# stefan01/Fusion-Method-for-Video-Frame-Interpolation

Measured on NVIDIA B200. Metric: interpolated_1080p_frames_per_s, higher is better.
Workload: dtype f32

## Files before the change

### fusion-method-for-video-frame-interpolation_b200/csrc/common.cuh

```cuda
#pragma once
#include <cuda_runtime.h>
#include <stdint.h>
#include <stdio.h>
#include <string>

#include "fvfi.h"

namespace fvfi {

void set_error(const char* fmt, ...);
void note_launch();

#define FVFI_CHECK_ARG(cond, ...)            \
    do {                                     \
        if (!(cond)) {                       \
            ::fvfi::set_error(__VA_ARGS__);  \
            return FVFI_EINVAL;              \
        }                                    \
    } while (0)

#define FVFI_CUDA(expr)                                                                   \
    do {                                                                                  \
        cudaError_t _e = (expr);                                                          \
        if (_e != cudaSuccess) {                                                          \
// ... 27 lines not shown
__host__ __device__ __forceinline__ int ceil_div(int a, int b) { return (a + b - 1) / b; }

__device__ __forceinline__ float ld_stream(const float* p) {
    float v;
    asm("ld.global.nc.L1::no_allocate.f32 %0, [%1];" : "=f"(v) : "l"(p));
    return v;
}
__device__ __forceinline__ void st_stream(float* p, float v) {
    asm volatile("st.global.L1::no_allocate.f32 [%0], %1;" ::"l"(p), "f"(v) : "memory");
}
__device__ __forceinline__ float4 ld_stream4(const float4* p) {
    float4 v;
    asm("ld.global.nc.L1::no_allocate.v4.f32 {%0,%1,%2,%3}, [%4];"
                 : "=f"(v.x), "=f"(v.y), "=f"(v.z), "=f"(v.w)
                 : "l"(p));
    return v;
}
__device__ __forceinline__ void st_stream4(float4* p, float4 v) {
    asm volatile("st.global.L1::no_allocate.v4.f32 [%0], {%1,%2,%3,%4};" ::"l"(p), "f"(v.x), "f"(v.y),
                 "f"(v.z), "f"(v.w)
                 : "memory");
}

__host__ __device__ __forceinline__ void bilinear_src(int o, float scale, int align_corners, int n_in, int& i0, int& i1, float& l) {
    const float f = align_corners ? scale * (float)o : fmaxf(scale * ((float)o + 0.5f) - 0.5f, 0.f);
    i0 = min((int)f, n_in - 1);
    i1 = min(i0 + 1, n_in - 1);
    l = f - (float)i0;
}
__host__ __device__ __forceinline__ float bilinear_scale(int n_in, int n_out, int align_corners) {
    if (align_corners) return n_out > 1 ? (float)(n_in - 1) / (float)(n_out - 1) : 0.f;
    return (float)n_in / (float)n_out;
}
__device__ __forceinline__ float bilerp(float hy, float hx, float ly, float lx, float a, float b, float c, float d) {
    return fmaf(ly, fmaf(lx, d, hx * c), hy * fmaf(lx, b, hx * a));
}
}
```

### fusion-method-for-video-frame-interpolation_b200/csrc/conv_tc.cu

```cuda
#include <cuda_fp16.h>

#include <algorithm>
#include <atomic>
#include <cstdlib>
#include <mutex>
#include <type_traits>

#include "common.cuh"

namespace fvfi {

constexpr int CV_KCHUNKS = 4;
constexpr int CV_UMAX = 12;
constexpr int CV_HDR = 32;
constexpr int CV_X_SHIFT = 4;
constexpr int CV_ROWS = 16;
constexpr int CV_LOADER_WARPS = 8;
constexpr int CV_LOADERS = 32 * CV_LOADER_WARPS;
constexpr int CV_EPI_WARPS = 4;
constexpr int CV_EPI_THREADS = 32 * CV_EPI_WARPS;
constexpr int CV_PRODUCER_WARP = CV_LOADER_WARPS + CV_EPI_WARPS;
constexpr int CV_MMA_WARP = CV_PRODUCER_WARP + 1;
constexpr int CV_THREADS = CV_LOADERS + CV_EPI_THREADS + 128;
constexpr int CV_REGS_LOADER = 152, CV_REGS_EPI = 144, CV_REGS_MISC = 56;
// ... 3 lines not shown
constexpr int CV_MAX_BSTAGES = 4;
constexpr unsigned CV_SPIN_LIMIT = 200u * 1000u * 1000u;

enum { ACT_NONE = 0, ACT_RELU = 1, ACT_ELU = 2, ACT_TANH = 3, ACT_SIGMOID = 4, ACT_SOFTMAX = 5 };
enum { PAD_ZERO = 0, PAD_REFLECT = 1 };
enum { PREC_TF32X3 = 0, PREC_F16X3 = 1 };
__host__ __device__ constexpr int cv_cpk(int prec) { return prec == PREC_F16X3 ? 8 : 4; }
__host__ __device__ constexpr int cv_chunk(int prec) { return CV_KCHUNKS * cv_cpk(prec); }

struct ConvArgs {
    const float* x;
    const float* wpack;
    const float* hdr;
    int* overflow;
    const float* bias;
    float* y;
    int B, H, W, Cin, Cout, Npad, KH, KW, pad_mode, act;
    int ldx, ldy;
    int out_nchw;
    int cout_store;
    int MT, RW, RH, NPIX;
    int KCS;
    int nchunks, last_ksteps, astages, bstages, tmem_cols;
    int wide, tcols;
    int nacc;
    int tiles_x, tiles_y, ntiles;
    unsigned a_stage_bytes, b_stage_bytes;
    const float* res;
    int ldr;
    int up, Hs, Ws, up_align;
    float up_sy, up_sx;
    const float* x2;
    int ldx2, up_chunks;
};

__device__ __forceinline__ unsigned smem_u32(const void* p) { return (unsigned)__cvta_generic_to_shared(p); }

__device__ __forceinline__ void mbar_init(unsigned long long* bar, unsigned count) {
    asm volatile("mbarrier.init.shared::cta.b64 [%0], %1;" ::"r"(smem_u32(bar)), "r"(count));
}
__device__ __forceinline__ void mbar_arrive(unsigned long long* bar) {
    asm volatile("mbarrier.arrive.shared::cta.b64 _, [%0];" ::"r"(smem_u32(bar)) : "memory");
}
__device__ __forceinline__ void mbar_expect_tx(unsigned long long* bar, unsigned bytes) {
    asm volatile("mbarrier.arrive.expect_tx.shared::cta.b64 _, [%0], %1;" ::"r"(smem_u32(bar)), "r"(bytes) : "memory");
}
__device__ __forceinline__ void mbar_wait(unsigned long long* bar, unsigned parity) {
    const unsigned addr = smem_u32(bar);
    unsigned done = 0, spins = 0;
    while (true) {
        asm volatile(
            "{\n\t.reg .pred p;\n\t"
            "mbarrier.try_wait.parity.shared::cta.b64 p, [%1], %2;\n\t"
            "selp.u32 %0, 1, 0, p;\n\t}"
            : "=r"(done)
            : "r"(addr), "r"(parity)
            : "memory");
        if (done) break;
        if (++spins > CV_SPIN_LIMIT) __trap();
    }
}
__device__ __forceinline__ void bulk_g2s(void* dst, const void* src, unsigned bytes, unsigned long long* bar) {
    asm volatile("cp.async.bulk.shared::cluster.global.mbarrier::complete_tx::bytes [%0], [%1], %2, [%3];" ::"r"(smem_u32(dst)),
                 "l"(src), "r"(bytes), "r"(smem_u32(bar))
                 : "memory");
}
// ... 69 lines not shown
__device__ __forceinline__ void tc_ld_wait() { asm volatile("tcgen05.wait::ld.sync.aligned;" ::: "memory"); }
__device__ __forceinline__ void tc_ld16(unsigned taddr, float* v) {
    unsigned r[16];
    asm volatile(
        "tcgen05.ld.sync.aligned.32x32b.x16.b32 {%0,%1,%2,%3,%4,%5,%6,%7,%8,%9,%10,%11,%12,%13,%14,%15}, [%16];"
        : "=r"(r[0]), "=r"(r[1]), "=r"(r[2]), "=r"(r[3]), "=r"(r[4]), "=r"(r[5]), "=r"(r[6]), "=r"(r[7]), "=r"(r[8]),
          "=r"(r[9]), "=r"(r[10]), "=r"(r[11]), "=r"(r[12]), "=r"(r[13]), "=r"(r[14]), "=r"(r[15])
        : "r"(taddr));
    asm volatile("tcgen05.wait::ld.sync.aligned;" ::: "memory");
#pragma unroll
    for (int i = 0; i < 16; ++i) v[i] = __uint_as_float(r[i]);
}

__device__ __forceinline__ unsigned long long make_desc(unsigned saddr, unsigned lbo_bytes, unsigned sbo_bytes) {
    unsigned long long d = 0;
    d |= (unsigned long long)((saddr >> 4) & 0x3fffu);
    d |= (unsigned long long)((lbo_bytes >> 4) & 0x3fffu) << 16;
    d |= (unsigned long long)((sbo_bytes >> 4) & 0x3fffu) << 32;
    d |= 1ull << 46;
    return d;
}

__device__ __forceinline__ void ldg256(const float* p, float* v) {
    asm volatile("ld.global.nc.v8.f32 {%0,%1,%2,%3,%4,%5,%6,%7}, [%8];"
                 : "=f"(v[0]), "=f"(v[1]), "=f"(v[2]), "=f"(v[3]), "=f"(v[4]), "=f"(v[5]), "=f"(v[6]), "=f"(v[7])
                 : "l"(p));
}
__device__ __forceinline__ void stg256(float* p, const float* v) {
    asm volatile("st.global.v8.f32 [%0], {%1,%2,%3,%4,%5,%6,%7,%8};" ::"l"(p), "f"(v[0]), "f"(v[1]), "f"(v[2]), "f"(v[3]),
                 "f"(v[4]), "f"(v[5]), "f"(v[6]), "f"(v[7])
                 : "memory");
}

__device__ __forceinline__ float to_tf32_rna(float x) {
    unsigned r;
    asm("cvt.rna.tf32.f32 %0, %1;" : "=r"(r) : "f"(x));
    return __uint_as_float(r);
}

__device__ __forceinline__ float fast_tanh(float v) {
    const float t = __expf(2.f * fminf(fmaxf(v, -15.f), 15.f));
    return __fdividef(t - 1.f, t + 1.f);
}
__device__ __forceinline__ float fast_sigmoid(float v) { return __fdividef(1.f, 1.f + __expf(-fmaxf(v, -80.f))); }
template <int ACT>
__device__ __forceinline__ float apply_act(float v) {
    switch (ACT) {
        case ACT_RELU: return fmaxf(v, 0.f);
        case ACT_ELU: return v > 0.f ? v : __expf(v) - 1.f;
        case ACT_TANH: return fast_tanh(v);
        case ACT_SIGMOID: return fast_sigmoid(v);
        default: return v;
    }
}

__device__ __forceinline__ int reflect101(int i, int n) {
    if (n == 1) return 0;
    const int period = 2 * (n - 1);
    int m = i % period;
    if (m < 0) m += period;
    return m < n ? m : period - m;
}

__global__ void conv_weight_scale_kernel(const float* __restrict__ w, size_t count, float* __restrict__ hdr, int prec) {
    __shared__ float red[32];
    float m = 0.f;
// ... 41 lines not shown
        size_t t = q;
        const int e = (int)(t % CPK); t /= CPK;
        const int n = (int)(t % Npad); t /= Npad;
        const int lo = (int)(t % 2); t /= 2;
        const int kc = (int)(t % CV_KCHUNKS); t /= CV_KCHUNKS;
        const int tap = (int)(t % taps); t /= taps;
        const int chunk = (int)t;
        const int c = chunk * (CV_KCHUNKS * CPK) + kc * CPK + e;
        float v = 0.f;
        if (n < Cout && c < Cin) v = w[(((size_t)n * Cin + c) * KH + tap / KW) * KW + tap % KW];
        if (PREC == PREC_F16X3) {
            v *= wscale;
            const __half hi = __float2half_rn(v);
            out16[q] = lo ? __float2half_rn(v - __half2float(hi)) : hi;
        } else {
            unsigned hb;
            asm("cvt.rna.tf32.f32 %0, %1;" : "=r"(hb) : "f"(v));
            const float hi = __uint_as_float(hb);
            out32[q] = lo ? (v - hi) : hi;
        }
    }
}

struct TileCoord { int img, y0, x0; };
__device__ __forceinline__ TileCoord tile_coord(const ConvArgs& A, int tile) {
    TileCoord t;
    const int bx = tile % A.tiles_x, r = tile / A.tiles_x;
    t.x0 = bx * 8 * A.MT;
    t.y0 = (r % A.tiles_y) * CV_ROWS;
    t.img = r / A.tiles_y;
    return t;
}

template <int ACT, int PREC>
__global__ void __launch_bounds__(CV_THREADS, 1) conv_split_kernel(const ConvArgs A) {
    extern __shared__ __align__(128) unsigned char smem_raw[];
    unsigned char* a_base = smem_raw;
    unsigned char* b_base = a_base + (size_t)A.astages * A.a_stage_bytes;
    unsigned long long* bars = (unsigned long long*)(b_base + (size_t)A.bstages * A.b_stage_bytes);
    unsigned long long* a_full = bars;
    unsigned long long* a_empty = bars + CV_MAX_ASTAGES;
    unsigned long long* b_full = bars + 2 * CV_MAX_ASTAGES;
    unsigned long long* b_empty = b_full + CV_MAX_BSTAGES;
    unsigned long long* acc_full = b_empty + CV_MAX_BSTAGES;
    unsigned long long* acc_empty = acc_full + 2;
    unsigned* tmem_ptr = (unsigned*)(acc_empty + 2);
    int* pixoff = (int*)(tmem_ptr + 2);
    float* bias_s = (float*)(((size_t)(pixoff + A.NPIX) + 15) & ~(size_t)15);
    float2* up_w = (float2*)(bias_s + 256);
    int* up_d = (int*)(up_w + A.NPIX);
    int* up_off = up_d + A.NPIX;

    const int warp = threadIdx.x >> 5, lane = threadIdx.x & 31;
    const int taps = A.KH * A.KW;
    const unsigned a_half = A.a_stage_bytes / 2;
    const int nacc = A.nacc;
    const unsigned acc_cols = (unsigned)(A.MT * A.tcols);

    if (threadIdx.x == 0) {
        for (int s = 0; s < A.astages; ++s) { mbar_init(&a_full[s], CV_LOADERS); mbar_init(&a_empty[s], 1); }
        for (int s = 0; s < A.bstages; ++s) { mbar_init(&b_full[s], 1); mbar_init(&b_empty[s], 1); }
        for (int s = 0; s < 2; ++s) { mbar_init(&acc_full[s], 1); mbar_init(&acc_empty[s], CV_EPI_THREADS); }
        asm volatile("fence.mbarrier_init.release.cluster;" ::: "memory");
    }
    for (int n = threadIdx.x; n < A.Npad; n += CV_THREADS) bias_s[n] = (A.bias && n < A.Cout) ? __ldg(A.bias + n) : 0.f;
    if (warp == CV_MMA_WARP) {
        asm volatile("tcgen05.alloc.cta_group::1.sync.aligned.shared::cta.b32 [%0], %1;" ::"r"(smem_u32(tmem_ptr)), "r"(A.tmem_cols));
        asm volatile("tcgen05.relinquish_alloc_permit.cta_group::1.sync.aligned;");
    }
    tc_fence_before();
    __syncthreads();
    tc_fence_after();
    const unsigned tmem = *tmem_ptr;

    if (warp >= CV_LOADER_WARPS && warp < CV_PRODUCER_WARP) {
        if (CV_REGS_EPI > CV_REGS_LAUNCH) asm volatile("setmaxnreg.inc.sync.aligned.u32 %0;" ::"n"(CV_REGS_EPI));
        else asm volatile("setmaxnreg.dec.sync.aligned.u32 %0;" ::"n"(CV_REGS_EPI));
        const float oscale = __ldg(A.hdr);
        const bool vec_out = (A.cout_store & 3) == 0 && (A.ldy & 3) == 0 && ((((size_t)A.y) & 15) == 0);
        const bool vec_out8 = (A.cout_store & 7) == 0 && (A.ldy & 7) == 0 && ((((size_t)A.y) & 31) == 0);
        const size_t plane = (size_t)A.H * A.W;
        const int quarter = warp & 3;
        const int m = quarter * 32 + lane;
        const bool res_vec = A.res && (A.Cout & 15) == 0 && (A.ldr & 7) == 0 && ((((size_t)A.res) & 31) == 0);
// ... 162 lines not shown
                    emit_at(a0, a1);
                    if (k + 1 < nblk) {
                        tc_ld_wait();
                        if (k + 2 < nblk) issue_at(a0, a1);
                        emit_at(b0, b1);
                    }
                }
            }
            tc_fence_before();
            mbar_arrive(&acc_empty[buf]);
        };

        {
            int j = 0;
            for (int tile = blockIdx.x; tile < A.ntiles; tile += gridDim.x, ++j) epilogue(j, tile_coord(A, tile));
        }
    } else if (warp < CV_LOADER_WARPS) {
        asm volatile("setmaxnreg.inc.sync.aligned.u32 %0;" ::"n"(CV_REGS_LOADER));
        const int padT = A.KH / 2, padL = A.KW / 2;
        constexpr int CPK = cv_cpk(PREC);
        constexpr int CHUNK = cv_chunk(PREC);
        const int cshift = A.up ? A.up_chunks * CHUNK : 0;
        const float* xd = (A.up && A.x2) ? A.x2 : A.x;
        const int ldd = (A.up && A.x2) ? A.ldx2 : A.ldx, cind = A.Cin - cshift;
        const int cin4 = (cind + 3) & ~3;
        const bool vec = ((ldd & 3) == 0) && (ldd >= cin4) && ((((size_t)xd) & 15) == 0);
        const int cin8 = (cind + 7) & ~7;
        const bool vec8 = ((ldd & 7) == 0) && (ldd >= cin8) && ((((size_t)xd) & 31) == 0);
        const int cin4u = A.up ? ((min(A.Cin, cshift) + 3) & ~3) : 0;
        const float xs = (float)(1 << CV_X_SHIFT);
        float amax = 0.f;
        int g = 0;

        constexpr int UMAX = CV_UMAX;
        float v[UMAX][CPK];
        auto chunk_shape = [&](int c, int& ksh) {
            ksh = (c == A.nchunks - 1 && A.last_ksteps == 1) ? 1 : 2;
            return A.NPIX << ksh;
        };
        auto issue = [&](int c, const float* X) {
            int ksh;
            const int total = chunk_shape(c, ksh);
            const int kmask = (1 << ksh) - 1, cbase = c * CHUNK - cshift;
#pragma unroll
            for (int u = 0; u < UMAX; ++u) {
                const int q = threadIdx.x + u * CV_LOADERS;
#pragma unroll
                for (int e = 0; e < CPK; ++e) v[u][e] = 0.f;
                if (q < total) {
                    const int pix = q >> ksh, ch = cbase + (q & kmask) * CPK;
                    const int off = pixoff[pix];
                    if (off >= 0 && ch < cin4) {
                        const float* p = X + (size_t)off * ldd + ch;
                        if (vec8 && CPK == 8 && ch + 8 <= cin8) {
                            ldg256(p, v[u]);
                        } else if (vec) {
#pragma unroll
                            for (int e = 0; e < CPK; e += 4) {
                                if (ch + e < cin4) {
                                    const float4 t = __ldg((const float4*)(p + e));
                                    v[u][e] = t.x; v[u][e + 1] = t.y; v[u][e + 2] = t.z; v[u][e + 3] = t.w;
                                }
                            }
                        } else {
#pragma unroll
                            for (int e = 0; e < CPK; ++e)
                                if (ch + e < cind) v[u][e] = __ldg(p + e);
                        }
                    }
                }
            }
        };
        auto finish = [&](int c) {
            const int s = g % A.astages;
            if (g >= A.astages) mbar_wait(&a_empty[s], ((g / A.astages) - 1) & 1);
            ++g;
            float4* hi = (float4*)(a_base + (size_t)s * A.a_stage_bytes);
            float4* lo = (float4*)(a_base + (size_t)s * A.a_stage_bytes + a_half);
            int ksh;
            const int total = chunk_shape(c, ksh);
            const int kmask = (1 << ksh) - 1;
#pragma unroll
            for (int u = 0; u < UMAX; ++u) {
                const int q = threadIdx.x + u * CV_LOADERS;
                if (q < total) {
                    const int o = (q & kmask) * A.KCS + (q >> ksh);
                    if (PREC == PREC_F16X3) {
                        unsigned hw[4], lw[4];
#pragma unroll
                        for (int e = 0; e < 8; e += 2) {
                            const float x0 = v[u][e] * xs, x1 = v[u][e + 1] * xs;
                            amax = fmaxf(amax, fmaxf(fabsf(x0), fabsf(x1)));
                            const __half2 h = __floats2half2_rn(x0, x1);
                            const float2 hf = __half22float2(h);
                            const __half2 l = __floats2half2_rn(x0 - hf.x, x1 - hf.y);
                            hw[e >> 1] = *(const unsigned*)&h;
                            lw[e >> 1] = *(const unsigned*)&l;
                        }
                        hi[o] = make_float4(__uint_as_float(hw[0]), __uint_as_float(hw[1]), __uint_as_float(hw[2]), __uint_as_float(hw[3]));
                        lo[o] = make_float4(__uint_as_float(lw[0]), __uint_as_float(lw[1]), __uint_as_float(lw[2]), __uint_as_float(lw[3]));
                    } else {
                        float4 h;
                        h.x = to_tf32_rna(v[u][0]); h.y = to_tf32_rna(v[u][1]); h.z = to_tf32_rna(v[u][2]); h.w = to_tf32_rna(v[u][3]);
                        hi[o] = h;
                        lo[o] = make_float4(v[u][0] - h.x, v[u][1] - h.y, v[u][2] - h.z, v[u][3] - h.w);
                    }
                }
            }
            fence_async_smem();
            mbar_arrive(&a_full[s]);
        };
        auto load_cpk = [&](const float* p, float* dst) {
            if (CPK == 8) {
                ldg256(p, dst);
            } else {
                const float4 t = __ldg((const float4*)p);
                dst[0] = t.x; dst[1] = t.y; dst[2] = t.z; dst[3] = t.w;
            }
        };
        auto stage_up = [&](int c, const float* X) {
            const int s = g % A.astages;
            if (g >= A.astages) mbar_wait(&a_empty[s], ((g / A.astages) - 1) & 1);
            ++g;
            float4* hi = (float4*)(a_base + (size_t)s * A.a_stage_bytes);
            float4* lo = (float4*)(a_base + (size_t)s * A.a_stage_bytes + a_half);
            int ksh;
            const int total = chunk_shape(c, ksh) >> 1;
            const int kmask = (1 << ksh) - 1, cbase = c * CHUNK;
            auto put = [&](int o, const float* w) {
                if (PREC == PREC_F16X3) {
                    unsigned hw[4], lw[4];
#pragma unroll
                    for (int e = 0; e < 8; e += 2) {
                        const float x0 = w[e] * xs, x1 = w[e + 1] * xs;
                        amax = fmaxf(amax, fmaxf(fabsf(x0), fabsf(x1)));
                        const __half2 h = __floats2half2_rn(x0, x1);
                        const float2 hf = __half22float2(h);
                        const __half2 l = __floats2half2_rn(x0 - hf.x, x1 - hf.y);
                        hw[e >> 1] = *(const unsigned*)&h;
                        lw[e >> 1] = *(const unsigned*)&l;
                    }
                    hi[o] = make_float4(__uint_as_float(hw[0]), __uint_as_float(hw[1]), __uint_as_float(hw[2]), __uint_as_float(hw[3]));
                    lo[o] = make_float4(__uint_as_float(lw[0]), __uint_as_float(lw[1]), __uint_as_float(lw[2]), __uint_as_float(lw[3]));
                } else {
                    float4 h;
                    h.x = to_tf32_rna(w[0]); h.y = to_tf32_rna(w[1]); h.z = to_tf32_rna(w[2]); h.w = to_tf32_rna(w[3]);
                    hi[o] = h;
                    lo[o] = make_float4(w[0] - h.x, w[1] - h.y, w[2] - h.z, w[3] - h.w);
                }
            };
            for (int q = threadIdx.x; q < total; q += CV_LOADERS) {
                const int pix = (q >> ksh) << 1, kg = q & kmask, ch = cbase + kg * CPK;
                float a0[CPK], b0[CPK], c0[CPK], d0[CPK], a1[CPK], b1[CPK], c1[CPK], d1[CPK];
#pragma unroll
                for (int e = 0; e < CPK; ++e) a0[e] = b0[e] = c0[e] = d0[e] = a1[e] = b1[e] = c1[e] = d1[e] = 0.f;
                const bool chok = ch < cin4u;
                const int off0 = chok ? up_off[pix] : -1, off1 = chok ? up_off[pix + 1] : -1;
                const int e0 = up_d[pix], e1 = up_d[pix + 1];
                const float2 w0 = up_w[pix], w1 = up_w[pix + 1];
                const int kind = (off0 >= 0 && off1 == off0 && e1 == e0) ? 0
                               : (off0 >= 0 && off1 == off0 + (e0 & 1) && (e1 >> 1) == (e0 >> 1)) ? 1 : 2;
                if (off0 >= 0) {
                    const float* p = X + (size_t)off0 * A.ldx + ch;
                    const size_t dx = (size_t)(e0 & 1) * A.ldx, dy = (size_t)(e0 >> 1) * A.ldx;
                    load_cpk(p, a0); load_cpk(p + dx, b0); load_cpk(p + dy, c0); load_cpk(p + dy + dx, d0);
                }
                if (off1 >= 0 && kind != 0) {
                    const float* p = X + (size_t)off1 * A.ldx + ch;
                    const size_t dx = (size_t)(e1 & 1) * A.ldx, dy = (size_t)(e1 >> 1) * A.ldx;
                    if (kind == 2) { load_cpk(p, a1); load_cpk(p + dy, c1); }
                    load_cpk(p + dx, b1); load_cpk(p + dy + dx, d1);
                }
                float w[CPK];
                {
                    const float ly = w0.x, lx = w0.y, hy = 1.f - ly, hx = 1.f - lx;
#pragma unroll
                    for (int e = 0; e < CPK; ++e) w[e] = bilerp(hy, hx, ly, lx, a0[e], b0[e], c0[e], d0[e]);
                    put(kg * A.KCS + pix, w);
                }
                {
                    const float ly = w1.x, lx = w1.y, hy = 1.f - ly, hx = 1.f - lx;
#pragma unroll
                    for (int e = 0; e < CPK; ++e) {
                        const float a = kind == 0 ? a0[e] : kind == 1 ? b0[e] : a1[e], cc = kind == 0 ? c0[e] : kind == 1 ? d0[e] : c1[e];
                        const float b = kind == 0 ? b0[e] : b1[e], d = kind == 0 ? d0[e] : d1[e];
                        w[e] = off1 >= 0 ? bilerp(hy, hx, ly, lx, a, b, cc, d) : 0.f;
                    }
                    put(kg * A.KCS + pix + 1, w);
                }
            }
            fence_async_smem();
            mbar_arrive(&a_full[s]);
        };
        auto map_tile = [&](const TileCoord& T) {
            asm volatile("bar.sync 1, %0;" ::"n"(CV_LOADERS) : "memory");
            for (int pix = threadIdx.x; pix < A.NPIX; pix += CV_LOADERS) {
                const int r = pix / A.RW, cc = pix - r * A.RW;
                int gy = T.y0 + r - padT, gx = T.x0 + cc - padL;
                bool ok = true;
                if (A.pad_mode == PAD_REFLECT) {
                    gy = reflect101(gy, A.H);
                    gx = reflect101(gx, A.W);
                } else {
                    ok = (gy >= 0 && gy < A.H && gx >= 0 && gx < A.W);
                }
                if (A.up) {
                    int y0 = 0, y1 = 0, x0 = 0, x1 = 0;
                    float ly = 0.f, lx = 0.f;
                    if (ok) {
                        bilinear_src(gy, A.up_sy, A.up_align, A.Hs, y0, y1, ly);
                        bilinear_src(gx, A.up_sx, A.up_align, A.Ws, x0, x1, lx);
                    }
                    up_off[pix] = ok ? y0 * A.Ws + x0 : -1;
                    up_w[pix] = make_float2(ly, lx);
                    up_d[pix] = ((y1 - y0) * A.Ws) * 2 + (x1 - x0);
                }
                pixoff[pix] = ok ? gy * A.W + gx : -1;
            }
            asm volatile("bar.sync 1, %0;" ::"n"(CV_LOADERS) : "memory");
        };

        TileCoord curT = tile_coord(A, blockIdx.x), nextT = curT;
        const float* X = xd + (size_t)curT.img * A.H * A.W * ldd;
        if (A.up) {
            for (int tile = blockIdx.x; tile < A.ntiles; tile += gridDim.x) {
                const TileCoord T = tile_coord(A, tile);
                const float* Xu = A.x + (size_t)T.img * A.Hs * A.Ws * A.ldx;
                X = xd + (size_t)T.img * A.H * A.W * ldd;
                map_tile(T);
                for (int c = 0; c < A.up_chunks; ++c) stage_up(c, Xu);
                for (int c = A.up_chunks; c < A.nchunks; ++c) {
                    issue(c, X);
                    finish(c);
                }
            }
        } else {
        if ((int)blockIdx.x < A.ntiles) {
            map_tile(curT);
            issue(0, X);
        }
        for (int tile = blockIdx.x; tile < A.ntiles; tile += gridDim.x) {
            for (int c = 0; c < A.nchunks; ++c) {
                finish(c);
                if (c + 1 < A.nchunks) {
                    issue(c + 1, X);
                } else if (tile + (int)gridDim.x < A.ntiles) {
                    nextT = tile_coord(A, tile + gridDim.x);
                    X = xd + (size_t)nextT.img * A.H * A.W * ldd;
                    map_tile(nextT);
                    issue(0, X);
                }
            }
            curT = nextT;
        }
        }
        if (PREC == PREC_F16X3 && !(amax <= 65504.f) && A.overflow) atomicOr(A.overflow, 1);
    } else {
      asm volatile("setmaxnreg.dec.sync.aligned.u32 %0;" ::"n"(CV_REGS_MISC));
      if (warp == CV_PRODUCER_WARP) {
        if (lane == 0) {
            int it = 0;
            for (int tile = blockIdx.x; tile < A.ntiles; tile += gridDim.x)
                for (int c = 0; c < A.nchunks; ++c)
                    for (int tp = 0; tp < taps; ++tp, ++it) {
                        const int s = it % A.bstages;
                        if (it >= A.bstages) mbar_wait(&b_empty[s], ((it / A.bstages) - 1) & 1);
// ... 74 lines not shown
        asm volatile("tcgen05.dealloc.cta_group::1.sync.aligned.b32 %0, %1;" ::"r"(tmem), "r"(A.tmem_cols));
    }
}

static int conv_geometry(ConvArgs& a, int prec, size_t* smem_bytes) {
    const int chunk = cv_chunk(prec);
    a.Npad = (a.Cout + 15) & ~15;
    FVFI_CHECK_ARG(a.Npad >= 16 && a.Npad <= 256, "conv: Cout %d not supported (1..256 per launch)", a.Cout);
    a.nchunks = (a.Cin + chunk - 1) / chunk;
    a.last_ksteps = (a.Cin - (a.nchunks - 1) * chunk) > chunk / 2 ? 2 : 1;
    a.b_stage_bytes = (unsigned)a.Npad * CV_KCHUNKS * 16u * 2u;
    const int taps = a.KH * a.KW;
    const size_t budget = 222 * 1024;
    static const int force_mt = [] { const char* e = getenv("FVFI_CONV_MT"); return e ? atoi(e) : 0; }();
    for (int mt = 4; mt >= 1; mt >>= 1) {
        if (force_mt && mt > force_mt) continue;
        a.wide = (a.Npad <= 32 && a.act != ACT_SOFTMAX) ? 1 : 0;
        a.tcols = a.wide ? 2 * a.Npad : a.Npad;
        if (mt * a.tcols > 512) continue;
        if (mt > 1 && 2 * mt * a.tcols > 512) continue;
        if (mt > 1 && 8 * (mt / 2) >= a.W) continue;
        a.MT = mt;
        a.nacc = (2 * mt * a.tcols <= 512) ? 2 : 1;
        a.RW = 8 * mt + a.KW - 1;
        a.RH = CV_ROWS + a.KH - 1;
        a.NPIX = a.RW * a.RH;
#ifdef FVFI_CONV_NO_KCS_PAD
        a.KCS = a.NPIX;
#else
        a.KCS = a.NPIX + ((2 - a.NPIX) & 7);
#endif
        a.a_stage_bytes = (unsigned)a.KCS * CV_KCHUNKS * 16u * 2u;
        if (a.NPIX * CV_KCHUNKS > CV_LOADERS * CV_UMAX) continue;
        const size_t misc = 512 + (size_t)a.NPIX * 4 + 1024 + 16 + (a.up ? (size_t)a.NPIX * 16 : 0);
        const int min_b = std::min(2, a.nchunks * taps);
        if (misc + 2 * (size_t)a.a_stage_bytes + (size_t)min_b * a.b_stage_bytes > budget) continue;
        int bs = std::min(CV_MAX_BSTAGES, std::max(min_b, (int)((budget - misc - 2 * (size_t)a.a_stage_bytes) / a.b_stage_bytes)));
        int as = (int)((budget - misc - (size_t)bs * a.b_stage_bytes) / a.a_stage_bytes);
        a.bstages = bs;
        a.astages = std::max(2, std::min(CV_MAX_ASTAGES, as));
        int cols = 32;
        while (cols < a.nacc * mt * a.tcols) cols <<= 1;
        a.tmem_cols = cols;
        *smem_bytes = misc + (size_t)a.astages * a.a_stage_bytes + (size_t)a.bstages * a.b_stage_bytes;
        a.tiles_x = ceil_div(a.W, 8 * mt);
        a.tiles_y = ceil_div(a.H, CV_ROWS);
        a.ntiles = a.tiles_x * a.tiles_y * a.B;
        return FVFI_OK;
    }
    set_error("conv: no tile configuration fits (Cout %d, kernel %dx%d)", a.Cout, a.KH, a.KW);
    return FVFI_EINVAL;
}

static int* overflow_flag() {
    static std::mutex mu;
    static std::atomic<int*> flags[FVFI_MAX_DEVICES];
    const int dev = current_device();
    if (dev < 0 || dev >= FVFI_MAX_DEVICES) return nullptr;
    int* p = flags[dev].load(std::memory_order_acquire);
    if (p) return p;
    std::lock_guard<std::mutex> lock(mu);
    p = flags[dev].load(std::memory_order_relaxed);
    if (!p) {
        if (cudaMalloc(&p, sizeof(int)) != cudaSuccess) return nullptr;
        cudaMemset(p, 0, sizeof(int));
        flags[dev].store(p, std::memory_order_release);
    }
    return p;
}

template <int PREC>
static void (*pick_kernel(int activation))(const ConvArgs) {
    switch (activation) {
        case ACT_RELU: return conv_split_kernel<ACT_RELU, PREC>;
        case ACT_ELU: return conv_split_kernel<ACT_ELU, PREC>;
        case ACT_TANH: return conv_split_kernel<ACT_TANH, PREC>;
        case ACT_SIGMOID: return conv_split_kernel<ACT_SIGMOID, PREC>;
        case ACT_SOFTMAX: return conv_split_kernel<ACT_SOFTMAX, PREC>;
        default: return conv_split_kernel<ACT_NONE, PREC>;
    }
}

}

using namespace fvfi;

extern "C" size_t fvfi_conv2d_packed_weight_floats(int Cout, int Cin, int KH, int KW, int precision) {
    const int Npad = (Cout + 15) & ~15;
    const int chunk = cv_chunk(precision);
    const int nchunks = (Cin + chunk - 1) / chunk;
    return (size_t)CV_HDR + (size_t)nchunks * KH * KW * 2 * CV_KCHUNKS * Npad * 4;
}

extern "C" int fvfi_conv2d_pack_weights(const float* weight_oihw, float* packed, int Cout, int Cin, int KH, int KW,
                                        int precision, void* stream) {
    FVFI_CHECK_ARG(weight_oihw && packed && Cout > 0 && Cin > 0 && KH > 0 && KW > 0, "conv_pack_weights: bad argument");
    FVFI_CHECK_ARG(precision == PREC_TF32X3 || precision == PREC_F16X3, "conv_pack_weights: precision must be 0 (3xTF32) or 1 (3xFP16)");
    const int Npad = (Cout + 15) & ~15;
    const int chunk = cv_chunk(precision);
    const int nchunks = (Cin + chunk - 1) / chunk;
    const size_t total = (size_t)nchunks * KH * KW * 2 * CV_KCHUNKS * Npad * cv_cpk(precision);
    const unsigned blocks = (unsigned)((total + 255) / 256 > 4096 ? 4096 : (total + 255) / 256);
    cudaStream_t s = (cudaStream_t)stream;
    conv_weight_scale_kernel<<<1, 1024, 0, s>>>(weight_oihw, (size_t)Cout * Cin * KH * KW, packed, precision);
    FVFI_LAUNCH_CHECK();
    if (precision == PREC_F16X3)
        conv_pack_weights_kernel<PREC_F16X3><<<blocks, 256, 0, s>>>(weight_oihw, packed, Cout, Cin, KH, KW, Npad, nchunks);
    else
        conv_pack_weights_kernel<PREC_TF32X3><<<blocks, 256, 0, s>>>(weight_oihw, packed, Cout, Cin, KH, KW, Npad, nchunks);
    FVFI_LAUNCH_CHECK();
    return FVFI_OK;
}
// ... 18 lines not shown
                                         const float* residual, int residual_pixel_stride, float* y, int y_pixel_stride, int B, int H,
                                         int W, int Cin, int Cout, int KH, int KW, int pad_mode, int activation, int out_nchw,
                                         int precision, void* stream) {
    return fvfi_conv2d_nhwc_upsampled(x, x_pixel_stride, 0, 0, 0, nullptr, 0, 0, packed_weight, bias, residual, residual_pixel_stride, y,
                                      y_pixel_stride, B, H, W, Cin, Cout, KH, KW, pad_mode, activation, out_nchw, precision, stream);
}

extern "C" int fvfi_conv2d_nhwc_upsampled(const float* x, int x_pixel_stride, int Hs, int Ws, int align_corners, const float* x_direct,
                                          int x_direct_pixel_stride, int cin_upsampled,
                                          const float* packed_weight, const float* bias, const float* residual,
                                          int residual_pixel_stride, float* y, int y_pixel_stride, int B, int H, int W, int Cin,
                                          int Cout, int KH, int KW, int pad_mode, int activation, int out_nchw, int precision,
                                          void* stream) {
    FVFI_CHECK_ARG(!residual || (activation != ACT_SOFTMAX && residual_pixel_stride >= Cout),
                   "conv2d: a residual needs a pixel stride >= Cout and no softmax");
    FVFI_CHECK_ARG(x && packed_weight && y, "conv2d: null pointer");
    FVFI_CHECK_ARG(B > 0 && H > 0 && W > 0 && Cin > 0 && Cout > 0 && B <= 65535, "conv2d: bad dimension");
    FVFI_CHECK_ARG((KH == 1 || KH == 3 || KH == 5) && KW == KH, "conv2d: kernel must be 1x1, 3x3 or 5x5");
    FVFI_CHECK_ARG(pad_mode == PAD_ZERO || pad_mode == PAD_REFLECT, "conv2d: pad_mode must be 0 (zero) or 1 (reflect)");
    FVFI_CHECK_ARG(pad_mode != PAD_REFLECT || (H > KH / 2 && W > KW / 2), "conv2d: reflect padding needs H,W > pad");
    FVFI_CHECK_ARG(activation >= 0 && activation <= 5, "conv2d: bad activation");
    FVFI_CHECK_ARG(activation != ACT_SOFTMAX || Cout <= 256, "conv2d: softmax needs all channels in one call");
    FVFI_CHECK_ARG(precision == PREC_TF32X3 || precision == PREC_F16X3, "conv2d: precision must be 0 (3xTF32) or 1 (3xFP16)");
    ConvArgs a{};
    a.x = x; a.hdr = packed_weight; a.wpack = packed_weight + CV_HDR; a.bias = bias; a.y = y;
    a.ldx = x_pixel_stride; a.ldy = y_pixel_stride; a.out_nchw = (out_nchw == 1) ? 1 : 0;
    a.res = residual; a.ldr = residual_pixel_stride;
    a.up = (Hs > 0 || Ws > 0) ? 1 : 0;
    if (a.up) {
        const int cpk = cv_cpk(precision), cin_r = (Cin + cpk - 1) / cpk * cpk;
        FVFI_CHECK_ARG(Hs > 0 && Ws > 0 && (size_t)Hs * Ws < (1u << 30), "conv2d: bad source size %dx%d for the upsampling loader", Hs, Ws);
        FVFI_CHECK_ARG((x_pixel_stride % cpk) == 0 && (x_direct || x_pixel_stride >= cin_r) && ((size_t)x % (4 * cpk)) == 0,
                       "conv2d: the upsampling loader needs an aligned source whose pixel stride is a multiple of %d and >= %d", cpk, cin_r);
        a.Hs = Hs; a.Ws = Ws; a.up_align = align_corners ? 1 : 0;
        a.up_sy = bilinear_scale(Hs, H, a.up_align);
        a.up_sx = bilinear_scale(Ws, W, a.up_align);
        const int chunk = cv_chunk(precision);
        a.up_chunks = (Cin + chunk - 1) / chunk;
        if (x_direct) {
            FVFI_CHECK_ARG(cin_upsampled > 0 && cin_upsampled < Cin && (cin_upsampled % chunk) == 0,
                           "conv2d: the upsampled part of a two-source input must be a multiple of %d channels (got %d of %d)", chunk,
                           cin_upsampled, Cin);
            FVFI_CHECK_ARG(x_direct_pixel_stride >= Cin - cin_upsampled, "conv2d: x_direct pixel stride smaller than its channel count");
            a.x2 = x_direct; a.ldx2 = x_direct_pixel_stride; a.up_chunks = cin_upsampled / chunk;
        }
    } else {
        FVFI_CHECK_ARG(!x_direct, "conv2d: x_direct needs an upsampled first source");
    }
    a.cout_store = (out_nchw == 2) ? ((Cout + 15) & ~15) : Cout;
    FVFI_CHECK_ARG(out_nchw >= 0 && out_nchw <= 2, "conv2d: output layout must be 0 (NHWC), 1 (NCHW) or 2 (NHWC, zero-padded channels)");
    FVFI_CHECK_ARG(out_nchw != 2 || y_pixel_stride >= a.cout_store, "conv2d: padded NHWC output needs a pixel stride >= round16(Cout)");
    a.overflow = (precision == PREC_F16X3) ? overflow_flag() : nullptr;
    FVFI_CHECK_ARG(x_pixel_stride >= (x_direct ? cin_upsampled : Cin) && (out_nchw || y_pixel_stride >= Cout),
                   "conv2d: pixel stride smaller than channel count");
    a.B = B; a.H = H; a.W = W; a.Cin = Cin; a.Cout = Cout; a.KH = KH; a.KW = KW; a.pad_mode = pad_mode; a.act = activation;
    size_t smem = 0;
    if (int rc = conv_geometry(a, precision, &smem)) return rc;
    const int nsm = sm_count();
    dim3 grid((unsigned)std::min(a.ntiles, nsm > 0 ? nsm : 148), 1, 1);
    void (*kern)(const ConvArgs) = (precision == PREC_F16X3) ? pick_kernel<PREC_F16X3>(activation) : pick_kernel<PREC_TF32X3>(activation);
    FVFI_SMEM_OPT_IN(kern, smem);
    kern<<<grid, CV_THREADS, smem, (cudaStream_t)stream>>>(a);
    FVFI_LAUNCH_CHECK();
    return FVFI_OK;
}
```

### fusion-method-for-video-frame-interpolation_b200/fvfi/conv.py

```python
import os

import torch

from . import _lib

PRECISIONS = {"tf32x3": 0, "f16x3": 1}
precision = PRECISIONS[os.environ.get("FVFI_CONV_PREC", "f16x3")]
range_check = True
_guard_depth = 0


def overflow_pending():
    import torch as _t
    _t.cuda.current_stream().synchronize()
    return _lib.lib().fvfi_conv2d_overflow_count() > 0


def check_overflow():
    if precision == PRECISIONS["f16x3"] and overflow_pending():
        raise FloatingPointError("fvfi.conv: activation beyond the 3xFP16 range (|x| > 4094); use conv.forced_precision('tf32x3')")


class forced_precision:

# ... 140 lines not shown
            return x
    return x.contiguous(memory_format=torch.channels_last)


fuse_upsample = True


def conv2d(x, weight, bias=None, padding_mode="zeros", act=None, out=None, nchw_out=False, pad_out=False, residual=None,
           upsample=None, x_direct=None):
    if not x.is_cuda:
        raise NotImplementedError("fvfi.conv.conv2d: CUDA tensors only")
    if torch.is_grad_enabled() and (x.requires_grad or weight.requires_grad or (bias is not None and bias.requires_grad)):
        assert upsample is None, "conv2d(upsample=...) is an inference form"
        assert out is None and not nchw_out and not pad_out and residual is None and act != "softmax", \
            "conv2d under autograd supports the plain NHWC form (bias + relu / elu / tanh / sigmoid)"
        return _ConvTC.apply(x, weight, bias, padding_mode, act)
    B, Cin, H, W = x.shape
    Cout, Cin_w, KH, KW = weight.shape
    xd, cin_up = None, 0
    if x_direct is not None:
        chunk = 32 if precision == PRECISIONS["f16x3"] else 16
        assert upsample is not None and Cin % chunk == 0 and Cin + x_direct.shape[1] >= Cin_w > Cin
        assert tuple(x_direct.shape[2:]) == tuple(int(v) for v in upsample[0]) and x_direct.shape[0] == B
        xd, cin_up = to_nhwc(x_direct.float()), Cin
        Cin = Cin_w
    assert Cin >= Cin_w and KH == KW and KH in (1, 3, 5)
    Cin = Cin_w
    xc = to_nhwc(x.float())
    assert xc.stride(1) == 1
    ldx = xc.stride(3)
    Hs = Ws = align = 0
    if upsample is not None:
        cpk = 8 if precision == PRECISIONS["f16x3"] else 4
        if ldx % cpk or ldx < ((cin_up or Cin) + cpk - 1) // cpk * cpk or xc.data_ptr() % (4 * cpk):
            up = resize_bilinear(xc, tuple(upsample[0]), bool(upsample[1]))
            if xd is not None:
                up = torch.cat((up[:, :cin_up], xd), 1)
            return conv2d(up, weight, bias, padding_mode, act, out, nchw_out, pad_out, residual)
        Hs, Ws, align = H, W, int(bool(upsample[1]))
        H, W = (int(v) for v in upsample[0])
    if (upsample is None and KH == 1 and Cout <= 8 and Cin % 8 == 0 and Cin <= 128 and ldx % 8 == 0 and xc.data_ptr() % 32 == 0
            and act != "softmax" and out is None and not nchw_out and not pad_out and residual is None):
        return _conv1x1_direct(xc, weight, bias, act)
    if out is None:
        out = torch.empty((B, (Cout + 15) // 16 * 16 if pad_out else Cout, H, W), dtype=torch.float32, device=x.device,
                          memory_format=torch.contiguous_format if nchw_out else torch.channels_last)
    ldy = Cout if nchw_out else out.stride(3)
    if nchw_out:
        assert out.is_contiguous() and Cout <= 256 and not pad_out
    if pad_out:
        assert Cout <= 256
    L = _lib.lib()
    pad_mode = {"zeros": 0, "reflect": 1}[padding_mode]
    b = None if bias is None else bias.detach().contiguous().float()
    rc = None
    if residual is not None:
        assert not nchw_out and act != "softmax" and tuple(residual.shape) == (B, Cout, H, W)
        rc = to_nhwc(residual.float())
    with torch.cuda.device(x.device):
        parts = _packed(weight)
        if timing is not None:
            e0, e1 = torch.cuda.Event(enable_timing=True), torch.cuda.Event(enable_timing=True)
            e0.record()
        for (o, n, buf) in parts:
            _lib.check(L.fvfi_conv2d_nhwc_upsampled(xc.data_ptr(), ldx, Hs, Ws, align, None if xd is None else xd.data_ptr(),
                                                    0 if xd is None else xd.stride(3), cin_up, buf.data_ptr(),
                                                    None if b is None else b.data_ptr() + 4 * o,
# ... 198 lines not shown
```

Before: 24.51.

## Restructure fused-upsample conv loader to walk column pairs down row strips reusing source rows

The bilinear-upsample loader in the tensor-core conv kernel is rewritten. The per-pixel offset and weight tables in shared memory are removed. Each loader thread now handles a pair of output columns over a strip of rows, caching horizontally interpolated source rows so they are reused across consecutive output rows, and prefetching the next rows into L1. The kernel is templated on UP, which shrinks the register array in the upsample variant, and the direct-channel chunks are issued in sub-batches. A new guard requires the source to be no larger than the output, otherwise it falls back to a separate resize.

New measurement: 24.85 (median of 6 runs). 1.4% higher.

```diff
diff --git a/fusion-method-for-video-frame-interpolation_b200/csrc/common.cuh b/fusion-method-for-video-frame-interpolation_b200/csrc/common.cuh
--- a/fusion-method-for-video-frame-interpolation_b200/csrc/common.cuh
+++ b/fusion-method-for-video-frame-interpolation_b200/csrc/common.cuh
@@ -83,7 +83,9 @@
     if (align_corners) return n_out > 1 ? (float)(n_in - 1) / (float)(n_out - 1) : 0.f;
     return (float)n_in / (float)n_out;
 }
+__device__ __forceinline__ float bilerp_row(float hx, float lx, float a, float b) { return fmaf(lx, b, hx * a); }
+__device__ __forceinline__ float bilerp_rows(float hy, float ly, float r0, float r1) { return fmaf(ly, r1, hy * r0); }
 __device__ __forceinline__ float bilerp(float hy, float hx, float ly, float lx, float a, float b, float c, float d) {
-    return fmaf(ly, fmaf(lx, d, hx * c), hy * fmaf(lx, b, hx * a));
+    return bilerp_rows(hy, ly, bilerp_row(hx, lx, a, b), bilerp_row(hx, lx, c, d));
 }
 }
diff --git a/fusion-method-for-video-frame-interpolation_b200/csrc/conv_tc.cu b/fusion-method-for-video-frame-interpolation_b200/csrc/conv_tc.cu
--- a/fusion-method-for-video-frame-interpolation_b200/csrc/conv_tc.cu
+++ b/fusion-method-for-video-frame-interpolation_b200/csrc/conv_tc.cu
@@ -59,6 +59,7 @@
     float up_sy, up_sx;
     const float* x2;
     int ldx2, up_chunks;
+    int up_seg, up_nseg;
 };
 
 __device__ __forceinline__ unsigned smem_u32(const void* p) { return (unsigned)__cvta_generic_to_shared(p); }
@@ -194,6 +195,8 @@
                  : "memory");
 }
 
+__device__ __forceinline__ void prefetch_l1(const float* p) { asm volatile("prefetch.global.L1 [%0];" ::"l"(p)); }
+
 __device__ __forceinline__ float to_tf32_rna(float x) {
     unsigned r;
     asm("cvt.rna.tf32.f32 %0, %1;" : "=r"(r) : "f"(x));
@@ -301,7 +304,7 @@
     return t;
 }
 
-template <int ACT, int PREC>
+template <int ACT, int PREC, bool UP>
 __global__ void __launch_bounds__(CV_THREADS, 1) conv_split_kernel(const ConvArgs A) {
     extern __shared__ __align__(128) unsigned char smem_raw[];
     unsigned char* a_base = smem_raw;
@@ -316,9 +319,6 @@
     unsigned* tmem_ptr = (unsigned*)(acc_empty + 2);
     int* pixoff = (int*)(tmem_ptr + 2);
     float* bias_s = (float*)(((size_t)(pixoff + A.NPIX) + 15) & ~(size_t)15);
-    float2* up_w = (float2*)(bias_s + 256);
-    int* up_d = (int*)(up_w + A.NPIX);
-    int* up_off = up_d + A.NPIX;
 
     const int warp = threadIdx.x >> 5, lane = threadIdx.x & 31;
     const int taps = A.KH * A.KW;
@@ -547,19 +547,19 @@
         float amax = 0.f;
         int g = 0;
 
-        constexpr int UMAX = CV_UMAX;
+        constexpr int UMAX = UP ? CV_UMAX / 2 : CV_UMAX;
         float v[UMAX][CPK];
         auto chunk_shape = [&](int c, int& ksh) {
             ksh = (c == A.nchunks - 1 && A.last_ksteps == 1) ? 1 : 2;
             return A.NPIX << ksh;
         };
-        auto issue = [&](int c, const float* X) {
+        auto issue = [&](int c, const float* X, int q0 = 0) {
             int ksh;
             const int total = chunk_shape(c, ksh);
             const int kmask = (1 << ksh) - 1, cbase = c * CHUNK - cshift;
 #pragma unroll
             for (int u = 0; u < UMAX; ++u) {
-                const int q = threadIdx.x + u * CV_LOADERS;
+                const int q = q0 + threadIdx.x + u * CV_LOADERS;
 #pragma unroll
                 for (int e = 0; e < CPK; ++e) v[u][e] = 0.f;
                 if (q < total) {
@@ -586,10 +586,34 @@
                 }
             }
         };
-        auto finish = [&](int c) {
-            const int s = g % A.astages;
-            if (g >= A.astages) mbar_wait(&a_empty[s], ((g / A.astages) - 1) & 1);
-            ++g;
+        auto put = [&](float4* hi, float4* lo, int o, const float* w) {
+            if (PREC == PREC_F16X3) {
+                unsigned hw[4], lw[4];
+#pragma unroll
+                for (int e = 0; e < 8; e += 2) {
+                    const float x0 = w[e] * xs, x1 = w[e + 1] * xs;
+                    amax = fmaxf(amax, fmaxf(fabsf(x0), fabsf(x1)));
+                    const __half2 h = __floats2half2_rn(x0, x1);
+                    const float2 hf = __half22float2(h);
+                    const __half2 l = __floats2half2_rn(x0 - hf.x, x1 - hf.y);
+                    hw[e >> 1] = *(const unsigned*)&h;
+                    lw[e >> 1] = *(const unsigned*)&l;
+                }
+                hi[o] = make_float4(__uint_as_float(hw[0]), __uint_as_float(hw[1]), __uint_as_float(hw[2]), __uint_as_float(hw[3]));
+                lo[o] = make_float4(__uint_as_float(lw[0]), __uint_as_float(lw[1]), __uint_as_float(lw[2]), __uint_as_float(lw[3]));
+            } else {
+                float4 h;
+                h.x = to_tf32_rna(w[0]); h.y = to_tf32_rna(w[1]); h.z = to_tf32_rna(w[2]); h.w = to_tf32_rna(w[3]);
+                hi[o] = h;
+                lo[o] = make_float4(w[0] - h.x, w[1] - h.y, w[2] - h.z, w[3] - h.w);
+            }
+        };
+        auto finish = [&](int c, int q0 = 0, bool first = true, bool last = true) {
+            if (first) {
+                if (g >= A.astages) mbar_wait(&a_empty[g % A.astages], ((g / A.astages) - 1) & 1);
+                ++g;
+            }
+            const int s = (g - 1) % A.astages;
             float4* hi = (float4*)(a_base + (size_t)s * A.a_stage_bytes);
             float4* lo = (float4*)(a_base + (size_t)s * A.a_stage_bytes + a_half);
             int ksh;
@@ -597,7 +621,7 @@
             const int kmask = (1 << ksh) - 1;
 #pragma unroll
             for (int u = 0; u < UMAX; ++u) {
-                const int q = threadIdx.x + u * CV_LOADERS;
+                const int q = q0 + threadIdx.x + u * CV_LOADERS;
                 if (q < total) {
                     const int o = (q & kmask) * A.KCS + (q >> ksh);
                     if (PREC == PREC_F16X3) {
@@ -622,8 +646,10 @@
                     }
                 }
             }
-            fence_async_smem();
-            mbar_arrive(&a_full[s]);
+            if (last) {
+                fence_async_smem();
+                mbar_arrive(&a_full[s]);
+            }
         };
         auto load_cpk = [&](const float* p, float* dst) {
             if (CPK == 8) {
@@ -633,77 +659,135 @@
                 dst[0] = t.x; dst[1] = t.y; dst[2] = t.z; dst[3] = t.w;
             }
         };
-        auto stage_up = [&](int c, const float* X) {
+        auto stage_up = [&](int c, const float* Xu, const TileCoord& T) {
             const int s = g % A.astages;
-            if (g >= A.astages) mbar_wait(&a_empty[s], ((g / A.astages) - 1) & 1);
+            const bool recycled = g >= A.astages;
+            const unsigned parity = ((g / A.astages) - 1) & 1;
             ++g;
+            bool have_slot = false;
+            auto slot = [&] {
+                if (!have_slot && recycled) mbar_wait(&a_empty[s], parity);
+                have_slot = true;
+            };
             float4* hi = (float4*)(a_base + (size_t)s * A.a_stage_bytes);
             float4* lo = (float4*)(a_base + (size_t)s * A.a_stage_bytes + a_half);
             int ksh;
-            const int total = chunk_shape(c, ksh) >> 1;
-            const int kmask = (1 << ksh) - 1, cbase = c * CHUNK;
-            auto put = [&](int o, const float* w) {
-                if (PREC == PREC_F16X3) {
-                    unsigned hw[4], lw[4];
-#pragma unroll
-                    for (int e = 0; e < 8; e += 2) {
-                        const float x0 = w[e] * xs, x1 = w[e + 1] * xs;
-                        amax = fmaxf(amax, fmaxf(fabsf(x0), fabsf(x1)));
-                        const __half2 h = __floats2half2_rn(x0, x1);
-                        const float2 hf = __half22float2(h);
-                        const __half2 l = __floats2half2_rn(x0 - hf.x, x1 - hf.y);
-                        hw[e >> 1] = *(const unsigned*)&h;
-                        lw[e >> 1] = *(const unsigned*)&l;
-                    }
-                    hi[o] = make_float4(__uint_as_float(hw[0]), __uint_as_float(hw[1]), __uint_as_float(hw[2]), __uint_as_float(hw[3]));
-                    lo[o] = make_float4(__uint_as_float(lw[0]), __uint_as_float(lw[1]), __uint_as_float(lw[2]), __uint_as_float(lw[3]));
+            chunk_shape(c, ksh);
+            const int kmask = (1 << ksh) - 1, npair = A.RW >> 1;
+            const int items = (npair * A.up_nseg) << ksh;
+            const size_t row_pitch = (size_t)A.Ws * A.ldx;
+            const float zero[CPK] = {};
+            auto src_row = [&](int r, int& y0, int& y1, float& ly) {
+                int gy = T.y0 + r - padT;
+                if (A.pad_mode == PAD_REFLECT) gy = reflect101(gy, A.H);
+                else if (gy < 0 || gy >= A.H) return false;
+                bilinear_src(gy, A.up_sy, A.up_align, A.Hs, y0, y1, ly);
+                return true;
+            };
+            for (int q = threadIdx.x; q < items; q += CV_LOADERS) {
+                const int kg = q & kmask, pr = (q >> ksh) % npair, seg = (q >> ksh) / npair;
+                const int ch = c * CHUNK + kg * CPK, cc = 2 * pr;
+                const int rbeg = seg * A.up_seg, rend = min(rbeg + A.up_seg, A.RH);
+                const int obase = kg * A.KCS + cc;
+                int gxa = T.x0 + cc - padL, gxb = gxa + 1;
+                bool oka = true, okb = true;
+                if (A.pad_mode == PAD_REFLECT) {
+                    gxa = reflect101(gxa, A.W);
+                    gxb = reflect101(gxb, A.W);
                 } else {
-                    float4 h;
-                    h.x = to_tf32_rna(w[0]); h.y = to_tf32_rna(w[1]); h.z = to_tf32_rna(w[2]); h.w = to_tf32_rna(w[3]);
-                    hi[o] = h;
-                    lo[o] = make_float4(w[0] - h.x, w[1] - h.y, w[2] - h.z, w[3] - h.w);
-                }
-            };
-            for (int q = threadIdx.x; q < total; q += CV_LOADERS) {
-                const int pix = (q >> ksh) << 1, kg = q & kmask, ch = cbase + kg * CPK;
-                float a0[CPK], b0[CPK], c0[CPK], d0[CPK], a1[CPK], b1[CPK], c1[CPK], d1[CPK];
-#pragma unroll
-                for (int e = 0; e < CPK; ++e) a0[e] = b0[e] = c0[e] = d0[e] = a1[e] = b1[e] = c1[e] = d1[e] = 0.f;
-                const bool chok = ch < cin4u;
-                const int off0 = chok ? up_off[pix] : -1, off1 = chok ? up_off[pix + 1] : -1;
-                const int e0 = up_d[pix], e1 = up_d[pix + 1];
-                const float2 w0 = up_w[pix], w1 = up_w[pix + 1];
-                const int kind = (off0 >= 0 && off1 == off0 && e1 == e0) ? 0
-                               : (off0 >= 0 && off1 == off0 + (e0 & 1) && (e1 >> 1) == (e0 >> 1)) ? 1 : 2;
-                if (off0 >= 0) {
-                    const float* p = X + (size_t)off0 * A.ldx + ch;
-                    const size_t dx = (size_t)(e0 & 1) * A.ldx, dy = (size_t)(e0 >> 1) * A.ldx;
-                    load_cpk(p, a0); load_cpk(p + dx, b0); load_cpk(p + dy, c0); load_cpk(p + dy + dx, d0);
-                }
-                if (off1 >= 0 && kind != 0) {
-                    const float* p = X + (size_t)off1 * A.ldx + ch;
-                    const size_t dx = (size_t)(e1 & 1) * A.ldx, dy = (size_t)(e1 >> 1) * A.ldx;
-                    if (kind == 2) { load_cpk(p, a1); load_cpk(p + dy, c1); }
-                    load_cpk(p + dx, b1); load_cpk(p + dy + dx, d1);
-                }
-                float w[CPK];
-                {
-                    const float ly = w0.x, lx = w0.y, hy = 1.f - ly, hx = 1.f - lx;
-#pragma unroll
-                    for (int e = 0; e < CPK; ++e) w[e] = bilerp(hy, hx, ly, lx, a0[e], b0[e], c0[e], d0[e]);
-                    put(kg * A.KCS + pix, w);
-                }
-                {
-                    const float ly = w1.x, lx = w1.y, hy = 1.f - ly, hx = 1.f - lx;
+                    oka = gxa >= 0 && gxa < A.W;
+                    okb = gxb >= 0 && gxb < A.W;
+                }
+                if (ch >= cin4u) oka = okb = false;
+                if (!oka && !okb) {
+                    slot();
+                    for (int r = rbeg; r < rend; ++r) {
+                        put(hi, lo, obase + r * A.RW, zero);
+                        put(hi, lo, obase + r * A.RW + 1, zero);
+                    }
+                    continue;
+                }
+                int xa0, xa1, xb0, xb1;
+                float lxa, lxb;
+                bilinear_src(oka ? gxa : gxb, A.up_sx, A.up_align, A.Ws, xa0, xa1, lxa);
+                bilinear_src(okb ? gxb : gxa, A.up_sx, A.up_align, A.Ws, xb0, xb1, lxb);
+                const float hxa = 1.f - lxa, hxb = 1.f - lxb;
+                const int xe = (xb1 != xa0 && xb1 != xa1) ? xb1 : xb0;
+                const int sb0 = xb0 == xa0 ? 0 : xb0 == xa1 ? 1 : 2, sb1 = xb1 == xa0 ? 0 : xb1 == xa1 ? 1 : 2;
+                const bool load_e = sb0 == 2 || sb1 == 2;
+                const float* base = Xu + ch;
+                auto load_row = [&](int sy, float (&v)[3][CPK]) {
+                    const float* p = base + (size_t)sy * row_pitch;
+                    load_cpk(p + (size_t)xa0 * A.ldx, v[0]);
+                    load_cpk(p + (size_t)xa1 * A.ldx, v[1]);
+                    if (load_e) load_cpk(p + (size_t)xe * A.ldx, v[2]);
+                };
+                auto lerp_row = [&](const float (&v)[3][CPK], float (&R)[2][CPK]) {
 #pragma unroll
                     for (int e = 0; e < CPK; ++e) {
-                        const float a = kind == 0 ? a0[e] : kind == 1 ? b0[e] : a1[e], cc = kind == 0 ? c0[e] : kind == 1 ? d0[e] : c1[e];
-                        const float b = kind == 0 ? b0[e] : b1[e], d = kind == 0 ? d0[e] : d1[e];
-                        w[e] = off1 >= 0 ? bilerp(hy, hx, ly, lx, a, b, cc, d) : 0.f;
-                    }
-                    put(kg * A.KCS + pix + 1, w);
+                        R[0][e] = bilerp_row(hxa, lxa, v[0][e], v[1][e]);
+                        const float b0 = sb0 == 0 ? v[0][e] : sb0 == 1 ? v[1][e] : v[2][e];
+                        const float b1 = sb1 == 0 ? v[0][e] : sb1 == 1 ? v[1][e] : v[2][e];
+                        R[1][e] = bilerp_row(hxb, lxb, b0, b1);
+                    }
+                };
+                float R0[2][CPK], R1[2][CPK];
+                int k0 = -1, k1 = -1;
+                auto request = [&](int y0, int y1) {
+                    auto pf = [&](int sy) {
+                        const float* p = base + (size_t)sy * row_pitch;
+                        prefetch_l1(p + (size_t)xa0 * A.ldx);
+                        prefetch_l1(p + (size_t)xa1 * A.ldx);
+                        if (load_e) prefetch_l1(p + (size_t)xe * A.ldx);
+                    };
+                    if (y0 != k0 && y0 != k1) pf(y0);
+                    if (y1 != k0 && y1 != k1 && y1 != y0) pf(y1);
+                };
+                auto fetch = [&](int y, float (&R)[2][CPK]) {
+                    float V[3][CPK];
+                    load_row(y, V);
+                    lerp_row(V, R);
+                };
+                auto settle = [&](int y0, int y1) {
+                    if (y0 == k1) {
+#pragma unroll
+                        for (int e = 0; e < CPK; ++e) { R0[0][e] = R1[0][e]; R0[1][e] = R1[1][e]; }
+                        k0 = k1;
+                    } else if (y0 != k0) {
+                        fetch(y0, R0);
+                        k0 = y0;
+                    }
+                    if (y1 == k1) return;
+                    if (y1 == k0) {
+#pragma unroll
+                        for (int e = 0; e < CPK; ++e) { R1[0][e] = R0[0][e]; R1[1][e] = R0[1][e]; }
+                    } else {
+                        fetch(y1, R1);
+                    }
+                    k1 = y1;
+                };
+                int y0 = 0, y1 = 0;
+                float ly = 0.f;
+                bool ok = src_row(rbeg, y0, y1, ly);
+                if (ok) request(y0, y1);
+                slot();
+                for (int r = rbeg; r < rend; ++r) {
+                    if (ok) settle(y0, y1);
+                    const bool okr = ok;
+                    const float hyr = 1.f - ly, lyr = ly;
+                    ok = r + 1 < rend && src_row(r + 1, y0, y1, ly);
+                    if (ok) request(y0, y1);
+                    const int o = obase + r * A.RW;
+                    float w[CPK];
+#pragma unroll
+                    for (int e = 0; e < CPK; ++e) w[e] = (okr && oka) ? bilerp_rows(hyr, lyr, R0[0][e], R1[0][e]) : 0.f;
+                    put(hi, lo, o, w);
+#pragma unroll
+                    for (int e = 0; e < CPK; ++e) w[e] = (okr && okb) ? bilerp_rows(hyr, lyr, R0[1][e], R1[1][e]) : 0.f;
+                    put(hi, lo, o + 1, w);
                 }
             }
+            slot();
             fence_async_smem();
             mbar_arrive(&a_full[s]);
         };
@@ -719,17 +803,6 @@
                 } else {
                     ok = (gy >= 0 && gy < A.H && gx >= 0 && gx < A.W);
                 }
-                if (A.up) {
-                    int y0 = 0, y1 = 0, x0 = 0, x1 = 0;
-                    float ly = 0.f, lx = 0.f;
-                    if (ok) {
-                        bilinear_src(gy, A.up_sy, A.up_align, A.Hs, y0, y1, ly);
-                        bilinear_src(gx, A.up_sx, A.up_align, A.Ws, x0, x1, lx);
-                    }
-                    up_off[pix] = ok ? y0 * A.Ws + x0 : -1;
-                    up_w[pix] = make_float2(ly, lx);
-                    up_d[pix] = ((y1 - y0) * A.Ws) * 2 + (x1 - x0);
-                }
                 pixoff[pix] = ok ? gy * A.W + gx : -1;
             }
             asm volatile("bar.sync 1, %0;" ::"n"(CV_LOADERS) : "memory");
@@ -737,16 +810,22 @@
 
         TileCoord curT = tile_coord(A, blockIdx.x), nextT = curT;
         const float* X = xd + (size_t)curT.img * A.H * A.W * ldd;
-        if (A.up) {
+        if (UP) {
             for (int tile = blockIdx.x; tile < A.ntiles; tile += gridDim.x) {
                 const TileCoord T = tile_coord(A, tile);
                 const float* Xu = A.x + (size_t)T.img * A.Hs * A.Ws * A.ldx;
-                X = xd + (size_t)T.img * A.H * A.W * ldd;
-                map_tile(T);
-                for (int c = 0; c < A.up_chunks; ++c) stage_up(c, Xu);
-                for (int c = A.up_chunks; c < A.nchunks; ++c) {
-                    issue(c, X);
-                    finish(c);
+                for (int c = 0; c < A.up_chunks; ++c) stage_up(c, Xu, T);
+                if (A.up_chunks < A.nchunks) {
+                    X = xd + (size_t)T.img * A.H * A.W * ldd;
+                    map_tile(T);
+                    for (int c = A.up_chunks; c < A.nchunks; ++c) {
+                        int ksh;
+                        const int total = chunk_shape(c, ksh);
+                        for (int q0 = 0; q0 < total; q0 += UMAX * CV_LOADERS) {
+                            issue(c, X, q0);
+                            finish(c, q0, q0 == 0, q0 + UMAX * CV_LOADERS >= total);
+                        }
+                    }
                 }
             }
         } else {
@@ -887,7 +966,7 @@
 #endif
         a.a_stage_bytes = (unsigned)a.KCS * CV_KCHUNKS * 16u * 2u;
         if (a.NPIX * CV_KCHUNKS > CV_LOADERS * CV_UMAX) continue;
-        const size_t misc = 512 + (size_t)a.NPIX * 4 + 1024 + 16 + (a.up ? (size_t)a.NPIX * 16 : 0);
+        const size_t misc = 512 + (size_t)a.NPIX * 4 + 1024 + 16;
         const int min_b = std::min(2, a.nchunks * taps);
         if (misc + 2 * (size_t)a.a_stage_bytes + (size_t)min_b * a.b_stage_bytes > budget) continue;
         int bs = std::min(CV_MAX_BSTAGES, std::max(min_b, (int)((budget - misc - 2 * (size_t)a.a_stage_bytes) / a.b_stage_bytes)));
@@ -898,6 +977,11 @@
         while (cols < a.nacc * mt * a.tcols) cols <<= 1;
         a.tmem_cols = cols;
         *smem_bytes = misc + (size_t)a.astages * a.a_stage_bytes + (size_t)a.bstages * a.b_stage_bytes;
+        if (a.up) {
+            const int strips = (a.RW / 2) * CV_KCHUNKS;
+            a.up_seg = ceil_div(a.RH, std::max(1, std::min(a.RH, CV_LOADERS / strips)));
+            a.up_nseg = ceil_div(a.RH, a.up_seg);
+        }
         a.tiles_x = ceil_div(a.W, 8 * mt);
         a.tiles_y = ceil_div(a.H, CV_ROWS);
         a.ntiles = a.tiles_x * a.tiles_y * a.B;
@@ -924,15 +1008,15 @@
     return p;
 }
 
-template <int PREC>
+template <int PREC, bool UP>
 static void (*pick_kernel(int activation))(const ConvArgs) {
     switch (activation) {
-        case ACT_RELU: return conv_split_kernel<ACT_RELU, PREC>;
-        case ACT_ELU: return conv_split_kernel<ACT_ELU, PREC>;
-        case ACT_TANH: return conv_split_kernel<ACT_TANH, PREC>;
-        case ACT_SIGMOID: return conv_split_kernel<ACT_SIGMOID, PREC>;
-        case ACT_SOFTMAX: return conv_split_kernel<ACT_SOFTMAX, PREC>;
-        default: return conv_split_kernel<ACT_NONE, PREC>;
+        case ACT_RELU: return conv_split_kernel<ACT_RELU, PREC, UP>;
+        case ACT_ELU: return conv_split_kernel<ACT_ELU, PREC, UP>;
+        case ACT_TANH: return conv_split_kernel<ACT_TANH, PREC, UP>;
+        case ACT_SIGMOID: return conv_split_kernel<ACT_SIGMOID, PREC, UP>;
+        case ACT_SOFTMAX: return conv_split_kernel<ACT_SOFTMAX, PREC, UP>;
+        default: return conv_split_kernel<ACT_NONE, PREC, UP>;
     }
 }
 
@@ -1017,6 +1101,8 @@
         FVFI_CHECK_ARG(Hs > 0 && Ws > 0 && (size_t)Hs * Ws < (1u << 30), "conv2d: bad source size %dx%d for the upsampling loader", Hs, Ws);
         FVFI_CHECK_ARG((x_pixel_stride % cpk) == 0 && (x_direct || x_pixel_stride >= cin_r) && ((size_t)x % (4 * cpk)) == 0,
                        "conv2d: the upsampling loader needs an aligned source whose pixel stride is a multiple of %d and >= %d", cpk, cin_r);
+        FVFI_CHECK_ARG(Hs <= H && Ws <= W, "conv2d: the upsampling loader needs a source no larger than the output (%dx%d -> %dx%d)",
+                       Hs, Ws, H, W);
         a.Hs = Hs; a.Ws = Ws; a.up_align = align_corners ? 1 : 0;
         a.up_sy = bilinear_scale(Hs, H, a.up_align);
         a.up_sx = bilinear_scale(Ws, W, a.up_align);
@@ -1043,7 +1129,9 @@
     if (int rc = conv_geometry(a, precision, &smem)) return rc;
     const int nsm = sm_count();
     dim3 grid((unsigned)std::min(a.ntiles, nsm > 0 ? nsm : 148), 1, 1);
-    void (*kern)(const ConvArgs) = (precision == PREC_F16X3) ? pick_kernel<PREC_F16X3>(activation) : pick_kernel<PREC_TF32X3>(activation);
+    void (*kern)(const ConvArgs) = (precision == PREC_F16X3)
+                                       ? (a.up ? pick_kernel<PREC_F16X3, true>(activation) : pick_kernel<PREC_F16X3, false>(activation))
+                                       : (a.up ? pick_kernel<PREC_TF32X3, true>(activation) : pick_kernel<PREC_TF32X3, false>(activation));
     FVFI_SMEM_OPT_IN(kern, smem);
     kern<<<grid, CV_THREADS, smem, (cudaStream_t)stream>>>(a);
     FVFI_LAUNCH_CHECK();
diff --git a/fusion-method-for-video-frame-interpolation_b200/fvfi/conv.py b/fusion-method-for-video-frame-interpolation_b200/fvfi/conv.py
--- a/fusion-method-for-video-frame-interpolation_b200/fvfi/conv.py
+++ b/fusion-method-for-video-frame-interpolation_b200/fvfi/conv.py
@@ -196,7 +196,8 @@
     Hs = Ws = align = 0
     if upsample is not None:
         cpk = 8 if precision == PRECISIONS["f16x3"] else 4
-        if ldx % cpk or ldx < ((cin_up or Cin) + cpk - 1) // cpk * cpk or xc.data_ptr() % (4 * cpk):
+        if (ldx % cpk or ldx < ((cin_up or Cin) + cpk - 1) // cpk * cpk or xc.data_ptr() % (4 * cpk)
+                or H > upsample[0][0] or W > upsample[0][1]):
             up = resize_bilinear(xc, tuple(upsample[0]), bool(upsample[1]))
             if xd is not None:
                 up = torch.cat((up[:, :cin_up], xd), 1)
```
